# myrrix/myrrix-recommender

Hardware: AMD Instinct MI355X
Metric: ALS rows solved/sec (full iteration) at k=64 (higher is better)
Workload: dtype f32 storage; per-row Gramian: f16x2-split operands (22 bits), f32 accumulate; Cholesky f32

## Files before the change

### myrrix-recommender_amd/csrc/als_kernels.h

```cpp
#pragma once
#include <hip/hip_runtime.h>
#include <stdint.h>

#include <type_traits>

namespace mals {

#ifndef MALS_WAVES
#define MALS_WAVES(T, MODE) ((T) <= 4 ? 4 : ((T) == 5 ? 3 : 2))
#endif
#ifndef MALS_WAVES_H
#define MALS_WAVES_H(T, MODE) ((T) <= 2 ? 5 : ((T) <= 4 ? 3 : 2))
#endif

typedef float f32x4 __attribute__((ext_vector_type(4)));
typedef double f64x4 __attribute__((ext_vector_type(4)));

__host__ __device__ constexpr int tri(int T) { return T * (T + 1) / 2; }
__host__ __device__ constexpr int tidx(int T, int i, int j) { return i * T - (i * (i - 1)) / 2 + (j - i); }

constexpr int GRAMIAN_FLUSH_BINADES = 5;
constexpr int YMAX_SLOTS = 64;

struct WorkItem {
  int64_t begin;
  int32_t len;
  int32_t id;
};
struct RowC {
  int64_t first_slot;
  int32_t row;
  int32_t nseg;
  int32_t stride;
  int32_t pad_;
};
constexpr int FINISH_GROUP = 32;

struct SolveParams {
  const int64_t* row_ptr;
  const int32_t* col;
  const float* val;
  const float* M;
  const float* Gf;
  const float* Gperm;
  float* out;
  const WorkItem* items;
  const RowC* rowsC;
  float* scratch;
  unsigned long long* bad_row;
  unsigned long long* suspect;
  int* any_marked;
  uint8_t* refine_flag;
  float refine_limit;
  float gramian_weight;
  int64_t n_work;
  int32_t k;
  int32_t ldm;
  int32_t flags;
  float alpha;
  float lambda_alpha;
  float sing_threshold;
  const float* zscale;
  unsigned long long* trace;
  int trace_start;
};

__device__ __forceinline__ float bperm(int byte_idx, float v) {
  return __int_as_float(__builtin_amdgcn_ds_bpermute(byte_idx, __float_as_int(v)));
}
__device__ __forceinline__ float readlane(float v, int lane) {
  return __int_as_float(__builtin_amdgcn_readlane(__float_as_int(v), lane));
}
__device__ __forceinline__ float select4(int q, float t0, float t1, float t2, float t3) {
  const bool b0 = q & 1, b1 = q & 2;
  const float lo = b0 ? t1 : t0, hi = b0 ? t3 : t2;
  return b1 ? hi : lo;
}
__device__ __forceinline__ int uniform(int v) { return __builtin_amdgcn_readfirstlane(v); }
__device__ __forceinline__ int64_t uniform64(int64_t v) {
  const unsigned lo = (unsigned)__builtin_amdgcn_readfirstlane((int)(unsigned)(v & 0xffffffffll));
  const int hi = __builtin_amdgcn_readfirstlane((int)(v >> 32));
  return ((int64_t)hi << 32) | lo;
}
template <int N>
__device__ __forceinline__ float row_ror(float v) {
  return __int_as_float(__builtin_amdgcn_update_dpp(0, __float_as_int(v), 0x120 + N, 0xf, 0xf, false));
}
template <int LANE>
__device__ __forceinline__ float row_bcast(float v) {
  return __int_as_float(__builtin_amdgcn_update_dpp(0, __float_as_int(v), 0x150 + LANE, 0xf, 0xf, false));
}
__device__ __forceinline__ float reduce_row16(float x) {
  x += row_ror<8>(x);
  x += row_ror<4>(x);
  x += row_ror<2>(x);
  x += row_ror<1>(x);
  return x;
}
#ifndef MALS_REDUCE_GROUPS_BPERM
#define MALS_REDUCE_GROUPS_BPERM 0
#endif
__device__ __forceinline__ float reduce_groups(float x, int lane) {
#if MALS_REDUCE_GROUPS_BPERM
  x += bperm((lane ^ 16) << 2, x);
  x += bperm((lane ^ 32) << 2, x);
  return x;
#else
  typedef unsigned u32x2 __attribute__((ext_vector_type(2)));
  const unsigned xi = __float_as_uint(x);
  const u32x2 a = __builtin_amdgcn_permlane32_swap(xi, xi, false, false);
  const float s = __uint_as_float(a[0]) + __uint_as_float(a[1]);
  const unsigned si = __float_as_uint(s);
  const u32x2 b = __builtin_amdgcn_permlane16_swap(si, si, false, false);
  return __uint_as_float(b[0]) + __uint_as_float(b[1]);
#endif
}
__device__ __forceinline__ f32x4 mfma4(float a, float b, f32x4 c) {
  return __builtin_amdgcn_mfma_f32_16x16x4f32(a, b, c, 0, 0, 0);
}

__device__ __forceinline__ f32x4 tile_ptq(const f32x4& P, const f32x4& Q, f32x4 C) {
  C = mfma4(P[0], Q[0], C);
  C = mfma4(P[1], Q[1], C);
  C = mfma4(P[2], Q[2], C);
  C = mfma4(P[3], Q[3], C);
  return C;
}
__device__ __forceinline__ f32x4 tile_neg_ptq(const f32x4& P, const f32x4& Q, f32x4 C) {
  C = mfma4(-P[0], Q[0], C);
  C = mfma4(-P[1], Q[1], C);
  C = mfma4(-P[2], Q[2], C);
  C = mfma4(-P[3], Q[3], C);
  return C;
}

__device__ __forceinline__ float spread_to_col(float v, int lane);
template <int T_>
__device__ __forceinline__ void diag_step(f32x4& D, f32x4& E, int lane, int pos, float& minpiv, float& piv, float& num) {
  constexpr int gm = T_ & 3, rm = T_ >> 2, P = 4 * gm + rm;
  constexpr int gn = (T_ + 1) & 3, rn = ((T_ + 1) >> 2) & 3, PN = 4 * gn + rn;
  const int c = lane & 15;
  const float rinv = __builtin_amdgcn_rcpf(piv);
  float nl = -(num * rinv);
  nl = pos > T_ ? nl : 0.f;
#define MALS_FMAC_BCAST(n, cond) ".if " cond "\n\tv_fmac_f32_dpp %" #n ", %" #n ", %8 row_newbcast:%9 row_mask:0xf bank_mask:0xf\n\t.endif\n\t"
  if constexpr (T_ < 15) {
    asm volatile(".if %10 == 0\n\ts_nop 1\n\t.endif\n\t"
                 MALS_FMAC_BCAST(0, "%11 == 0") MALS_FMAC_BCAST(1, "%11 == 1") MALS_FMAC_BCAST(2, "%11 == 2") MALS_FMAC_BCAST(3, "%11 == 3")
                 : "+v"(D[0]), "+v"(D[1]), "+v"(D[2]), "+v"(D[3]), "+v"(E[0]), "+v"(E[1]), "+v"(E[2]), "+v"(E[3])
                 : "v"(nl), "n"(P), "n"(T_), "n"(rn));
    __builtin_amdgcn_sched_barrier(0);
    num = bperm(((16 * gn) | c) << 2, D[rn]);
    piv = readlane(D[rn], 16 * gn + PN);
    __builtin_amdgcn_sched_barrier(0);
    asm volatile(MALS_FMAC_BCAST(0, "(3 > %10) && (%11 != 0)") MALS_FMAC_BCAST(1, "(7 > %10) && (%11 != 1)")
                 MALS_FMAC_BCAST(2, "(11 > %10) && (%11 != 2)") MALS_FMAC_BCAST(3, "(15 > %10) && (%11 != 3)")
                 MALS_FMAC_BCAST(4, "0 <= %10") MALS_FMAC_BCAST(5, "4 <= %10") MALS_FMAC_BCAST(6, "8 <= %10") MALS_FMAC_BCAST(7, "12 <= %10")
                 : "+v"(D[0]), "+v"(D[1]), "+v"(D[2]), "+v"(D[3]), "+v"(E[0]), "+v"(E[1]), "+v"(E[2]), "+v"(E[3])
                 : "v"(nl), "n"(P), "n"(T_), "n"(rn));
  } else {
    asm volatile(MALS_FMAC_BCAST(4, "0 <= %10") MALS_FMAC_BCAST(5, "4 <= %10") MALS_FMAC_BCAST(6, "8 <= %10") MALS_FMAC_BCAST(7, "12 <= %10")
                 : "+v"(D[0]), "+v"(D[1]), "+v"(D[2]), "+v"(D[3]), "+v"(E[0]), "+v"(E[1]), "+v"(E[2]), "+v"(E[3])
                 : "v"(nl), "n"(P), "n"(T_), "n"(rn));
  }
#undef MALS_FMAC_BCAST
}

__device__ __forceinline__ f32x4 factor_diag(f32x4 D, int lane, float& minpiv) {
  const int g = lane >> 4, c = lane & 15;
  const int pos = 4 * (c & 3) + (c >> 2);
  f32x4 E;
#pragma unroll
  for (int r = 0; r < 4; ++r) E[r] = (4 * g + r == c) ? 1.f : 0.f;
  float num = bperm(c << 2, D[0]);
  float piv = readlane(D[0], 0);
  diag_step<0>(D, E, lane, pos, minpiv, piv, num);
  diag_step<1>(D, E, lane, pos, minpiv, piv, num);
  diag_step<2>(D, E, lane, pos, minpiv, piv, num);
  diag_step<3>(D, E, lane, pos, minpiv, piv, num);
  diag_step<4>(D, E, lane, pos, minpiv, piv, num);
  diag_step<5>(D, E, lane, pos, minpiv, piv, num);
  diag_step<6>(D, E, lane, pos, minpiv, piv, num);
  diag_step<7>(D, E, lane, pos, minpiv, piv, num);
  diag_step<8>(D, E, lane, pos, minpiv, piv, num);
  diag_step<9>(D, E, lane, pos, minpiv, piv, num);
  diag_step<10>(D, E, lane, pos, minpiv, piv, num);
  diag_step<11>(D, E, lane, pos, minpiv, piv, num);
  diag_step<12>(D, E, lane, pos, minpiv, piv, num);
  diag_step<13>(D, E, lane, pos, minpiv, piv, num);
  diag_step<14>(D, E, lane, pos, minpiv, piv, num);
  diag_step<15>(D, E, lane, pos, minpiv, piv, num);
  const float pvc = spread_to_col(select4(c & 3, D[0], D[1], D[2], D[3]), lane);
  minpiv = fminf(minpiv, pvc == pvc ? pvc : 0.f);
  const float s = __builtin_amdgcn_rsqf(pvc);
#pragma unroll
  for (int r = 0; r < 4; ++r) E[r] *= s;
  return E;
}

typedef _Float16 f16x4h __attribute__((ext_vector_type(4)));
typedef int i32x2h __attribute__((ext_vector_type(2)));
struct TileH {
  i32x2h h, l;
};
__device__ __forceinline__ int pk_rn16(float a, float b) {
  typedef float f32x2r __attribute__((ext_vector_type(2)));
  typedef _Float16 f16x2r __attribute__((ext_vector_type(2)));
  const f32x2r v = {a, b};
  return __builtin_bit_cast(int, __builtin_convertvector(v, f16x2r));
}
__device__ __forceinline__ float residual_lo(int h, float z) {
  float o;
  asm("v_fma_mix_f32 %0, %1, -1.0, %2 op_sel:[0,0,0] op_sel_hi:[1,0,0]" : "=v"(o) : "v"(h), "v"(z));
  return o;
}
__device__ __forceinline__ float residual_hi(int h, float z) {
  float o;
  asm("v_fma_mix_f32 %0, %1, -1.0, %2 op_sel:[1,0,0] op_sel_hi:[1,0,0]" : "=v"(o) : "v"(h), "v"(z));
  return o;
}

__device__ __forceinline__ TileH split_tile(const f32x4& t) {
  const int h01 = pk_rn16(t[0], t[1]), h23 = pk_rn16(t[2], t[3]);
  const int l01 = pk_rn16(residual_lo(h01, t[0]), residual_hi(h01, t[1]));
  const int l23 = pk_rn16(residual_lo(h23, t[2]), residual_hi(h23, t[3]));
  TileH o;
  o.h[0] = h01;
  o.h[1] = h23;
  o.l[0] = l01;
  o.l[1] = l23;
  return o;
}
__device__ __forceinline__ TileH negate_tile(const TileH& t) {
  TileH o;
  o.h = t.h ^ (int)0x80008000;
  o.l = t.l ^ (int)0x80008000;
  return o;
}
__device__ __forceinline__ f32x4 mfma16h(const i32x2h& a, const i32x2h& b, f32x4 c) {
  return __builtin_amdgcn_mfma_f32_16x16x16f16(__builtin_bit_cast(f16x4h, a), __builtin_bit_cast(f16x4h, b), c, 0, 0, 0);
}
__device__ __forceinline__ f32x4 tile_ptq_h(const TileH& P, const TileH& Q, f32x4 C) {
  C = mfma16h(P.h, Q.h, C);
// ... 231 lines not shown
      "ds_bpermute_b32 %0, %4, %5 offset:%7\n\t"
      "ds_bpermute_b32 %1, %4, %5 offset:%8\n\t"
      "ds_bpermute_b32 %2, %4, %6 offset:%7\n\t"
      "ds_bpermute_b32 %3, %4, %6 offset:%8\n\t"
      "s_waitcnt lgkmcnt(0)"
      : "=&v"(a0), "=&v"(a1), "=&v"(b0), "=&v"(b1)
      : "v"(addr), "v"(a), "v"(b), "n"(O0), "n"(O1));
}
template <int O0, int O1>
__device__ __forceinline__ void bperm2_i_start(int addr, int v, int& r0, int& r1) {
  asm volatile(
      "ds_bpermute_b32 %0, %2, %3 offset:%4\n\t"
      "ds_bpermute_b32 %1, %2, %3 offset:%5"
      : "=&v"(r0), "=&v"(r1)
      : "v"(addr), "v"(v), "n"(O0), "n"(O1));
}
__device__ __forceinline__ void bperm2_i_land(int& r0, int& r1) {
  asm volatile("s_waitcnt lgkmcnt(0)" : "+v"(r0), "+v"(r1));
}
template <int O0, int O1>
__device__ __forceinline__ void bperm2_i(int addr, int v, int& r0, int& r1) {
  asm volatile(
      "ds_bpermute_b32 %0, %2, %3 offset:%4\n\t"
      "ds_bpermute_b32 %1, %2, %3 offset:%5\n\t"
      "s_waitcnt lgkmcnt(0)"
      : "=&v"(r0), "=&v"(r1)
      : "v"(addr), "v"(v), "n"(O0), "n"(O1));
}

template <bool ROWMAJOR = false>
__device__ __forceinline__ Chunk chunk_issue(const SolveParams& p, int64_t begin, int len, int base, int lane) {
  const int n = base + (ROWMAJOR ? (((lane & 15) << 2) | (lane >> 4)) : lane);
  const int nn = n < len ? n : len - 1;
  Chunk e;
  e.col = __builtin_nontemporal_load(p.col + begin + nn);
  e.w = __builtin_nontemporal_load(p.val + begin + nn);
  e.cb = n < len ? 1.f : 0.f;
  return e;
}
__device__ __forceinline__ void chunk_weights(const SolveParams& p, Chunk& e) {
  const float r = e.w, ok = e.cb;
  const float base_w = (p.flags & 2) ? 1.f : 0.f;
  float w, cb;
  if (p.flags & 1) {
    w = base_w;
    cb = r;
  } else {
    const float ar = p.alpha * fabsf(r);
    w = base_w + ar;
    cb = r > 0.f ? 1.f + ar : 0.f;
  }
  e.w = ok * w;
  e.cb = ok * cb;
}

template <int T>
__device__ __forceinline__ void load_rows(const float* __restrict__ M, int ldm, int col, int c, float (&y)[T]) {
  const float* p = M + ((uint64_t)(uint32_t)col * (uint32_t)ldm + (uint32_t)c);
#pragma unroll
  for (int v = 0; v < T; ++v) y[v] = p[16 * v];
}

template <int T>
__device__ __forceinline__ void gram_step(const float (&y)[T], float w, float cb, f32x4 (&acc)[tri(T)], float (&bpart)[T]) {
  float a[T];
#pragma unroll
  for (int v = 0; v < T; ++v) a[v] = w * y[v];
#pragma unroll
  for (int i = 0; i < T; ++i)
#pragma unroll
    for (int j = i; j < T; ++j) acc[tidx(T, i, j)] = mfma4(a[i], y[j], acc[tidx(T, i, j)]);
#pragma unroll
  for (int v = 0; v < T; ++v) bpart[v] = fmaf(cb, y[v], bpart[v]);
}

template <int T, int D>
struct Pipe {
  Chunk ch;
  float y[D][T];
  float wcur, cbcur;
  int colpf;
};

template <int T, int D, bool FULL>
__device__ __forceinline__ void prime_row(const SolveParams& p, int lane, Pipe<T, D>& pp) {
  const int c = lane & 15, gb = (lane >> 4) << 2;
#pragma unroll
  for (int i = 0; i < D - 1; ++i) load_rows<T>(p.M, p.ldm, bperm_i(gb + 16 * i, pp.ch.col), c, pp.y[i]);
  pp.wcur = bperm(gb, pp.ch.w);
  pp.cbcur = bperm(gb, pp.ch.cb);
  pp.colpf = bperm_i(gb + 16 * (D - 1), pp.ch.col);
}

template <int T, int D, bool FULL>
__device__ __forceinline__ void gather_row(const SolveParams& p, int64_t begin, int len, int lane, Pipe<T, D>& pp,
                                           f32x4 (&acc)[tri(T)], float (&bpart)[T]) {
  static_assert(16 % D == 0, "ring depth must divide the chunk length in steps");
  const int c = lane & 15, gb = (lane >> 4) << 2;
  const int nsteps = (len + 3) >> 2;
  for (int q = 0; 16 * q < nsteps; ++q) {
    Chunk chn = chunk_issue(p, begin, len, 64 * (q + 1), lane);
#pragma unroll
    for (int j = 0; j < 16; ++j) {
      const int s = 16 * q + j;
      if (s < nsteps) {
        load_rows<T>(p.M, p.ldm, pp.colpf, c, pp.y[(j + D - 1) % D]);
        __builtin_amdgcn_sched_barrier(0);
        if (j == 14) chunk_weights(p, chn);
        const int jn = j + 1, jt = j + D;
        const float wn = bperm(gb + 16 * (jn & 15), jn < 16 ? pp.ch.w : chn.w);
        const float cbn = bperm(gb + 16 * (jn & 15), jn < 16 ? pp.ch.cb : chn.cb);
        const int coln = bperm_i(gb + 16 * (jt & 15), jt < 16 ? pp.ch.col : chn.col);
        gram_step<T>(pp.y[j % D], pp.wcur, pp.cbcur, acc, bpart);
        pp.wcur = wn;
        pp.cbcur = cbn;
        pp.colpf = coln;
        __builtin_amdgcn_sched_barrier(0);
      }
    }
    pp.ch = chn;
  }
}

typedef _Float16 f16x8 __attribute__((ext_vector_type(8)));
typedef _Float16 f16x4 __attribute__((ext_vector_type(4)));
typedef _Float16 f16x2 __attribute__((ext_vector_type(2)));
typedef int i32x4 __attribute__((ext_vector_type(4)));
typedef int i32x2 __attribute__((ext_vector_type(2)));

template <int E>
struct ZOp {
  int r[E / 2];
};
template <int E>
__device__ __forceinline__ f32x4 mfma_h(const ZOp<E>& a, const ZOp<E>& b, f32x4 c) {
  if constexpr (E == 8) {
    return __builtin_amdgcn_mfma_f32_16x16x32_f16(__builtin_bit_cast(f16x8, a), __builtin_bit_cast(f16x8, b), c, 0, 0, 0);
  } else {
    return __builtin_amdgcn_mfma_f32_16x16x16f16(__builtin_bit_cast(f16x4, a), __builtin_bit_cast(f16x4, b), c, 0, 0, 0);
  }
}
#ifndef MALS_SPLIT8_MAXT
#define MALS_SPLIT8_MAXT 7
#endif
__host__ __device__ constexpr int split_slots(int T) { return T <= MALS_SPLIT8_MAXT ? 8 : 4; }

__device__ __forceinline__ void chunk_weights_h(const SolveParams& p, Chunk& e, float zscale) {
  chunk_weights(p, e);
  e.w = __builtin_amdgcn_sqrtf(e.w) * zscale;
}

template <int T, int E, bool FULL, int E2>
__device__ __forceinline__ void issue_pair_h(const SolveParams& p, int col_src, int off, int lane, float (&raw)[T][E]) {
  const int c = lane & 15;
  int col[2];
  bperm2_i<8 * E2, 8 * E2 + 4>(off, col_src, col[0], col[1]);
#ifdef MALS_PROFILING
  if (p.flags & 0x400) {
    col[0] &= 0xfff;
    col[1] &= 0xfff;
  }
#endif
#pragma unroll
  for (int i = 0; i < 2; ++i) {
    const int e = 2 * E2 + i;
    const float* ptr = p.M + ((uint64_t)(uint32_t)col[i] * (uint32_t)p.ldm + (uint32_t)c);
#pragma unroll
    for (int v = 0; v < T; ++v) raw[v][e] = ptr[16 * v];
  }
}

template <int E2>
__device__ __forceinline__ void fetch_pair_cols_h(int col_src, int off, int (&col)[2]) {
  bperm2_i_start<8 * E2, 8 * E2 + 4>(off, col_src, col[0], col[1]);
}
template <int T, int E, bool FULL, int E2>
__device__ __forceinline__ void issue_pair_loads_h(const SolveParams& p, int (&col)[2], int lane, float (&raw)[T][E]) {
  const int c = lane & 15;
  bperm2_i_land(col[0], col[1]);
#ifdef MALS_PROFILING
  if (p.flags & 0x400) {
    col[0] &= 0xfff;
    col[1] &= 0xfff;
  }
#endif
#pragma unroll
  for (int i = 0; i < 2; ++i) {
    const int e = 2 * E2 + i;
    const float* ptr = p.M + ((uint64_t)(uint32_t)col[i] * (uint32_t)p.ldm + (uint32_t)c);
#pragma unroll
    for (int v = 0; v < T; ++v) raw[v][e] = ptr[16 * v];
  }
}

template <int T, int E, bool FULL, int PART, int E2, int NTERM = 2>
__device__ __forceinline__ void convert_pair_h(const SolveParams& p, const Chunk& ch, int lane, const float (&raw)[T][E], ZOp<E> (&zh)[T],
                                               ZOp<E> (&zl)[T], float (&bpart)[T], ZOp<E> (&zm)[NTERM == 3 ? T : 1]) {
  constexpr int m0 = E * PART + 2 * E2;
  const float s0 = row_bcast<m0>(ch.w), s1 = row_bcast<m0 + 1>(ch.w);
  const float c0 = row_bcast<m0>(ch.cb), c1 = row_bcast<m0 + 1>(ch.cb);
#pragma unroll
  for (int v = 0; v < T; ++v) {
    const float y0 = raw[v][2 * E2], y1 = raw[v][2 * E2 + 1];
    const float z0 = y0 * s0, z1 = y1 * s1;
    const int hp = pk_rn16(z0, z1);
    const f16x2 hh = __builtin_bit_cast(f16x2, hp);
    zh[v].r[E2] = hp;
    if constexpr (NTERM == 3) {
      const float r0 = fmaf((float)hh[0], -1.f, z0), r1 = fmaf((float)hh[1], -1.f, z1);
      const int mp = pk_rn16(r0, r1);
      const f16x2 mh = __builtin_bit_cast(f16x2, mp);
      zm[v].r[E2] = mp;
      zl[v].r[E2] = pk_rn16(fmaf((float)mh[0], -1.f, r0), fmaf((float)mh[1], -1.f, r1));
    } else {
      zl[v].r[E2] = pk_rn16(fmaf((float)hh[0], -1.f, z0), fmaf((float)hh[1], -1.f, z1));
    }
    bpart[v] = fmaf(c0, y0, bpart[v]);
    bpart[v] = fmaf(c1, y1, bpart[v]);
  }
}

template <int T, int E, bool FULL, int PART, int NTERM = 2>
__device__ __forceinline__ void convert_refill_h(const SolveParams& p, const Chunk& ch, int next_col, int next_off, int lane,
                                                 float (&raw)[T][E], ZOp<E> (&zh)[T], ZOp<E> (&zl)[T], float (&bpart)[T], ZOp<E> (&zm)[NTERM == 3 ? T : 1]) {
#define MALS_SB __builtin_amdgcn_sched_barrier(0)
  int col[2];
  fetch_pair_cols_h<0>(next_col, next_off, col);
  MALS_SB;
  convert_pair_h<T, E, FULL, PART, 0, NTERM>(p, ch, lane, raw, zh, zl, bpart, zm);
  MALS_SB;
  issue_pair_loads_h<T, E, FULL, 0>(p, col, lane, raw);
  fetch_pair_cols_h<1>(next_col, next_off, col);
  MALS_SB;
  convert_pair_h<T, E, FULL, PART, 1, NTERM>(p, ch, lane, raw, zh, zl, bpart, zm);
  MALS_SB;
  issue_pair_loads_h<T, E, FULL, 1>(p, col, lane, raw);
  if constexpr (E == 8) {
    fetch_pair_cols_h<2>(next_col, next_off, col);
    MALS_SB;
    convert_pair_h<T, E, FULL, PART, 2, NTERM>(p, ch, lane, raw, zh, zl, bpart, zm);
    MALS_SB;
    issue_pair_loads_h<T, E, FULL, 2>(p, col, lane, raw);
    fetch_pair_cols_h<3>(next_col, next_off, col);
    MALS_SB;
    convert_pair_h<T, E, FULL, PART, 3, NTERM>(p, ch, lane, raw, zh, zl, bpart, zm);
    MALS_SB;
    issue_pair_loads_h<T, E, FULL, 3>(p, col, lane, raw);
  }
#undef MALS_SB
}

template <int T, int E>
__device__ __forceinline__ void gram_super_step(const ZOp<E> (&zh)[T], const ZOp<E> (&zl)[T], f32x4 (&acc)[tri(T)]) {
#pragma unroll
  for (int i = 0; i < T; ++i)
#pragma unroll
    for (int j = i; j < T; ++j) acc[tidx(T, i, j)] = mfma_h<E>(zh[i], zh[j], acc[tidx(T, i, j)]);
#pragma unroll
  for (int i = 0; i < T; ++i)
#pragma unroll
    for (int j = i; j < T; ++j) acc[tidx(T, i, j)] = mfma_h<E>(zh[i], zl[j], acc[tidx(T, i, j)]);
#pragma unroll
  for (int i = 0; i < T; ++i)
#pragma unroll
    for (int j = i; j < T; ++j) acc[tidx(T, i, j)] = mfma_h<E>(zl[i], zh[j], acc[tidx(T, i, j)]);
}

template <int T, int E>
__device__ __forceinline__ void gram_super_step3(const ZOp<E> (&zh)[T], const ZOp<E> (&zm)[T], const ZOp<E> (&zl)[T], f32x4 (&acc)[tri(T)]) {
#define MALS_GS3(A, B)                                                                                    \
  _Pragma("unroll") for (int i = 0; i < T; ++i) _Pragma("unroll") for (int j = i; j < T; ++j)              \
      acc[tidx(T, i, j)] = mfma_h<E>(A[i], B[j], acc[tidx(T, i, j)])
  MALS_GS3(zl, zh);
  MALS_GS3(zh, zl);
  MALS_GS3(zm, zm);
  MALS_GS3(zm, zh);
  MALS_GS3(zh, zm);
  MALS_GS3(zh, zh);
#undef MALS_GS3
}

template <int T, int E, bool FULL>
__device__ __forceinline__ void prime_row_h(const SolveParams& p, int col_src, int lane, float (&raw)[T][E]) {
  const int rb = (lane & 48) << 2;
  issue_pair_h<T, E, FULL, 0>(p, col_src, rb, lane, raw);
  issue_pair_h<T, E, FULL, 1>(p, col_src, rb, lane, raw);
  if constexpr (E == 8) {
    issue_pair_h<T, E, FULL, 2>(p, col_src, rb, lane, raw);
    issue_pair_h<T, E, FULL, 3>(p, col_src, rb, lane, raw);
  }
}

template <int T, int E, bool FULL, int PART, int NTERM = 2>
__device__ __forceinline__ void super_step_h(const SolveParams& p, const Chunk& ch, const Chunk& chn, int next_col, bool last, int lane,
                                             float (&raw)[T][E], f32x4 (&acc)[tri(T)], float (&bpart)[T]) {
  constexpr int NP = 16 / E;
  const int rb = (lane & 48) << 2;
  ZOp<E> zh[T], zl[T], zm[NTERM == 3 ? T : 1];
  const int same_row_col = PART == NP - 1 ? chn.col : ch.col;
  const int same_row_off = PART == NP - 1 ? rb : rb + 4 * E * (PART + 1);
  convert_refill_h<T, E, FULL, PART, NTERM>(p, ch, last ? next_col : same_row_col, last ? rb : same_row_off, lane, raw, zh, zl, bpart, zm);
  __builtin_amdgcn_sched_barrier(0);
  if constexpr (NTERM == 3) gram_super_step3<T, E>(zh, zm, zl, acc);
  else gram_super_step<T, E>(zh, zl, acc);
  __builtin_amdgcn_sched_barrier(0);
}

template <int T, int E, bool FULL, int NTERM = 2>
__device__ __forceinline__ void gather_row_h(const SolveParams& p, int64_t begin, int len, int lane, float zscale, Chunk& ch,
                                             int next_col, float (&raw)[T][E], f32x4 (&acc)[tri(T)], float (&bpart)[T]) {
  constexpr int NS = 4 * E, NP = 16 / E;
  const int n_ss = (len + NS - 1) / NS;
  for (int q = 0; NP * q < n_ss; ++q) {
    Chunk chn = chunk_issue<true>(p, begin, len, 64 * (q + 1), lane);
    const int ss = NP * q;
    super_step_h<T, E, FULL, 0, NTERM>(p, ch, chn, next_col, ss + 1 >= n_ss, lane, raw, acc, bpart);
    if (ss + 1 < n_ss) {
      if (NP == 2) chunk_weights_h(p, chn, zscale);
      super_step_h<T, E, FULL, 1, NTERM>(p, ch, chn, next_col, ss + 2 >= n_ss, lane, raw, acc, bpart);
    }
    if constexpr (NP == 4) {
      if (ss + 2 < n_ss) super_step_h<T, E, FULL, 2, NTERM>(p, ch, chn, next_col, ss + 3 >= n_ss, lane, raw, acc, bpart);
      if (ss + 3 < n_ss) {
        chunk_weights_h(p, chn, zscale);
        super_step_h<T, E, FULL, 3, NTERM>(p, ch, chn, next_col, ss + 4 >= n_ss, lane, raw, acc, bpart);
      }
    }
    ch = chn;
  }
}

template <int T>
__device__ __forceinline__ void init_acc(const SolveParams& p, f32x4 (&acc)[tri(T)], int lane) {
  if (!(p.flags & 2)) {
    const f32x4* G4 = reinterpret_cast<const f32x4*>(p.Gf) + lane;
#pragma unroll
    for (int t = 0; t < tri(T); ++t) acc[t] = G4[t * 64];
  } else {
#pragma unroll
    for (int t = 0; t < tri(T); ++t) acc[t] = f32x4{0.f, 0.f, 0.f, 0.f};
  }
}

template <int T, bool FULL = false>
__device__ __forceinline__ void add_ridge(const SolveParams& p, f32x4 (&acc)[tri(T)], int n_u, int lane) {
  const int g = lane >> 4, c = lane & 15;
  const float ridge = p.lambda_alpha * (float)n_u;
  float rd[4];
#pragma unroll
  for (int r = 0; r < 4; ++r) rd[r] = (4 * g + r == c) ? ridge : 0.f;
  float w00 = 1.f;
  if constexpr (!FULL) w00 = readlane(acc[tidx(T, 0, 0)][0], 0) + ridge;
#pragma unroll
  for (int v = 0; v < T; ++v) {
    if (FULL || v < T - 1) {
#pragma unroll
      for (int r = 0; r < 4; ++r) acc[tidx(T, v, v)][r] += rd[r];
    } else {
      const int feat = 16 * v + c;
#pragma unroll
      for (int r = 0; r < 4; ++r) {
        if (4 * g + r == c) acc[tidx(T, v, v)][r] = feat < p.k ? acc[tidx(T, v, v)][r] + ridge : w00;
      }
    }
  }
}

__device__ __forceinline__ int wave_max_bits(float mf, int lane) {
  int m = __float_as_int(mf);
  m = max(m, __builtin_amdgcn_update_dpp(0, m, 0x120 + 8, 0xf, 0xf, false));
  m = max(m, __builtin_amdgcn_update_dpp(0, m, 0x120 + 4, 0xf, 0xf, false));
  m = max(m, __builtin_amdgcn_update_dpp(0, m, 0x120 + 2, 0xf, 0xf, false));
  m = max(m, __builtin_amdgcn_update_dpp(0, m, 0x120 + 1, 0xf, 0xf, false));
  m = max(m, bperm_i((lane ^ 16) << 2, m));
  m = max(m, bperm_i((lane ^ 32) << 2, m));
  return m;
}
template <int T>
__device__ __forceinline__ int max_entry_bits(const f32x4 (&acc)[tri(T)], int lane) {
  float mf = 0.f;
#pragma unroll
  for (int v = 0; v < T; ++v) {
    const f32x4& d = acc[tidx(T, v, v)];
    mf = fmaxf(mf, fmaxf(fmaxf(fabsf(d[0]), fabsf(d[1])), fmaxf(fabsf(d[2]), fabsf(d[3]))));
  }
  return wave_max_bits(mf, lane);
}

template <int T>
__device__ __forceinline__ float row_part_max(const f32x4 (&acc)[tri(T)], const f32x4* gimg, int lane) {
  float mf = 0.f;
#pragma unroll
  for (int v = 0; v < T; ++v) {
    const f32x4 d = acc[tidx(T, v, v)] - gimg[tidx(T, v, v) * 64 + lane];
    mf = fmaxf(mf, fmaxf(fmaxf(fabsf(d[0]), fabsf(d[1])), fmaxf(fabsf(d[2]), fabsf(d[3]))));
  }
  return __int_as_float(wave_max_bits(mf, lane));
}

#ifndef MALS_PK_MAXT
#define MALS_PK_MAXT 7
#endif
template <int T>
__device__ __forceinline__ float row_scale(f32x4 (&acc)[tri(T)], float (&bcol)[T], int lane, float& wmax) {
  const int m = max_entry_bits<T>(acc, lane);
  wmax = __int_as_float(m);
  const int e = ((m >> 23) & 255) - 126;
  int p2 = 2 * (13 - ((e + 1) >> 1));
  p2 = p2 < -100 ? -100 : (p2 > 100 ? 100 : p2);
  const float s2 = __int_as_float((p2 + 127) << 23), inv_s2 = __int_as_float((127 - p2) << 23);
#pragma unroll
  for (int t = 0; t < tri(T); ++t) {
    if constexpr (T <= MALS_PK_MAXT) {
      acc[t] = acc[t] * s2;
    } else {
#pragma unroll
      for (int r = 0; r < 4; ++r) acc[t][r] *= s2;
    }
  }
#pragma unroll
  for (int v = 0; v < T; ++v) bcol[v] *= s2;
  return inv_s2;
}

template <int T, bool PERM = false>
__device__ __forceinline__ void store_row(const SolveParams& p, float (&xcol)[T], float minpiv, float wmax, int row, int lane) {
  if (!(minpiv > p.sing_threshold)) {
    if (lane == 0) {
      if (p.refine_flag) {
        p.refine_flag[row] = 2;
        *p.any_marked = 1;
      } else {
        atomicMin(p.bad_row, (unsigned long long)row);
      }
    }
#pragma unroll
    for (int v = 0; v < T; ++v) xcol[v] = 0.f;
  } else {
    if (minpiv <= 1024.f * p.sing_threshold && lane == 0) {
      const unsigned long long key = ((unsigned long long)__float_as_uint(minpiv) << 32) | (unsigned)row;
      if (key < __builtin_nontemporal_load(p.suspect)) atomicMin(p.suspect, key);
    }
    if (p.refine_flag && p.refine_limit > 0.f && wmax > p.refine_limit * minpiv && lane == 0) {
      p.refine_flag[row] = 1;
      *p.any_marked = 1;
    }
  }
  if constexpr (PERM) {
    static_assert(T == 8, "the permuted feature order belongs to the k = 128 kernels");
    float* o = p.out + (int64_t)row * p.k;
    int l2 = lane;
    asm volatile("" : "+v"(l2));
    const int g = l2 >> 4, c = l2 & 15;
    const bool hi = ((g ^ (c >> 3)) & 1) != 0;
    f32x4 x;
#pragma unroll
    for (int q = 0; q < 4; ++q) x[q] = hi ? xcol[4 + q] : xcol[q];
    if (g < 2) *reinterpret_cast<f32x4*>(o + 8 * c + 4 * g) = x;
  } else {
    float* o = p.out + (int64_t)row * p.k;
    int l2 = lane;
    asm volatile("" : "+v"(l2));
    const int g = l2 >> 4, c = l2 & 15;
#pragma unroll
    for (int m = 0; 4 * m < T; ++m) {
      const float x = select4(g, xcol[4 * m], 4 * m + 1 < T ? xcol[4 * m + 1] : 0.f, 4 * m + 2 < T ? xcol[4 * m + 2] : 0.f,
                              4 * m + 3 < T ? xcol[4 * m + 3] : 0.f);
      const int feat = 16 * (4 * m + g) + c;
      if (4 * m + 3 < T - 1 || feat < p.k) o[feat] = x;
    }
  }
}

template <int T, bool PERM = false>
__device__ __forceinline__ void finish_row(const SolveParams& p, f32x4 (&acc)[tri(T)], const float (&bcol)[T],
                                           int n_u, int row, int lane, float rmax = 0.f) {
  add_ridge<T, PERM>(p, acc, n_u, lane);
  float minpiv = 3.0e38f;
  float xcol[T];
  const float wmax = fmaxf(rmax, p.gramian_weight * __int_as_float(max_entry_bits<T>(acc, lane)));
  cholesky_tiles<T>(acc, lane, minpiv);
  solve_tiles<T>(acc, bcol, xcol, lane);
  store_row<T, PERM>(p, xcol, minpiv, wmax, row, lane);
}

__device__ __forceinline__ WorkItem load_item(const SolveParams& p, int64_t it) {
  WorkItem w;
  if (it < p.n_work) {
    w = p.items[it];
  } else {
    w.begin = 0;
    w.len = -1;
    w.id = 0;
  }
  return w;
}

template <int T, int D, int MODE, bool FULL>
__global__ __launch_bounds__(256, MALS_WAVES(T, MODE)) void als_persistent_kernel(SolveParams p) {
  __shared__ f32x4 sG[MODE == 0 ? tri(T) * 64 : 1];
  const int lane = threadIdx.x & 63;
  const int wave = uniform(blockIdx.x * 4 + (threadIdx.x >> 6));
  const int64_t n_waves = (int64_t)gridDim.x * 4;
  if (MODE == 0) {
    const f32x4* G4 = reinterpret_cast<const f32x4*>(p.Gf);
    for (int e = threadIdx.x; e < tri(T) * 64; e += 256) sG[e] = (p.flags & 2) ? f32x4{0.f, 0.f, 0.f, 0.f} : G4[e];
    __syncthreads();
  }
  int64_t it = wave;
  if (it >= p.n_work) return;
  if ((p.flags & 8) && p.zscale[2] != 0.f) return;
  WorkItem cur = load_item(p, it);
  WorkItem nxt = load_item(p, it + n_waves);
  Pipe<T, D> pp;
  pp.wcur = pp.cbcur = 0.f;
  pp.colpf = 0;
  pp.ch.col = 0;
  pp.ch.w = pp.ch.cb = 0.f;
#pragma unroll
  for (int i = 0; i < D; ++i)
#pragma unroll
    for (int v = 0; v < T; ++v) pp.y[i][v] = 0.f;
  if (cur.len > 0) {
    pp.ch = chunk_issue(p, cur.begin, cur.len, 0, lane);
    chunk_weights(p, pp.ch);
    prime_row<T, D, FULL>(p, lane, pp);
  }
  for (;;) {
    f32x4 acc[tri(T)];
    if (MODE == 0) {
#pragma unroll
      for (int t = 0; t < tri(T); ++t) acc[t] = sG[t * 64 + lane];
    } else {
#pragma unroll
      for (int t = 0; t < tri(T); ++t) acc[t] = f32x4{0.f, 0.f, 0.f, 0.f};
    }
    float bpart[T];
#pragma unroll
    for (int v = 0; v < T; ++v) bpart[v] = 0.f;
#ifdef MALS_PROFILING
    const int64_t trow = it / n_waves - p.trace_start;
    const bool tr = MODE == 0 && p.trace && wave < 64 && trow >= 0 && trow < 64;
    unsigned long long t0 = 0, t1 = 0, t2 = 0, t3 = 0;
    if (tr) t0 = __builtin_readcyclecounter();
    if (!(p.flags & 0x200)) gather_row<T, D, FULL>(p, cur.begin, cur.len, lane, pp, acc, bpart);
    if (tr) t1 = __builtin_readcyclecounter();
#else
    gather_row<T, D, FULL>(p, cur.begin, cur.len, lane, pp, acc, bpart);
#endif
    float bcol[T];
#pragma unroll
    for (int v = 0; v < T; ++v) bcol[v] = reduce_groups(bpart[v], lane);
    const bool prime_next = nxt.len > 0;
    if (prime_next) pp.ch = chunk_issue(p, nxt.begin, nxt.len, 0, lane);
    const WorkItem nxt2 = load_item(p, it + 2 * n_waves);
    if (MODE == 0) {
      const float wmax = p.refine_flag ? fmaxf(row_part_max<T>(acc, sG, lane), p.gramian_weight * __int_as_float(max_entry_bits<T>(acc, lane))) : 0.f;
      add_ridge<T, FULL>(p, acc, cur.len, lane);
      float minpiv = 3.0e38f;
      float xcol[T];
#ifdef MALS_PROFILING
      if (p.flags & 0x100) {
#pragma unroll
        for (int v = 0; v < T; ++v) xcol[v] = 1e-3f + 1e-9f * (bcol[v] + acc[tidx(T, v, v)][0] + acc[tidx(T, 0, v)][1]);
        if (prime_next) {
          chunk_weights(p, pp.ch);
          prime_row<T, D, FULL>(p, lane, pp);
        }
      } else
#endif
      {
        cholesky_tiles<T>(acc, lane, minpiv);
#ifdef MALS_PROFILING
        if (tr) t2 = __builtin_readcyclecounter();
#endif
        if (prime_next) {
          chunk_weights(p, pp.ch);
          prime_row<T, D, FULL>(p, lane, pp);
        }
        solve_tiles<T>(acc, bcol, xcol, lane);
      }
      store_row<T>(p, xcol, minpiv, wmax, cur.id, lane);
#ifdef MALS_PROFILING
      if (tr) {
        t3 = __builtin_readcyclecounter();
        if (lane == 0) {
          unsigned long long* o = p.trace + (trow * 64 + wave) * 6;
          o[0] = t0; o[1] = t1; o[2] = t2; o[3] = t3; o[4] = (unsigned long long)cur.len; o[5] = wall_clock64();
        }
      }
#endif
    } else {
      float* s = p.scratch + (int64_t)cur.id * ((tri(T) * 4 + T) * 64);
#pragma unroll
      for (int t = 0; t < tri(T); ++t) reinterpret_cast<f32x4*>(s)[t * 64 + lane] = acc[t];
#pragma unroll
      for (int v = 0; v < T; ++v) s[(tri(T) * 4 + v) * 64 + lane] = bcol[v];
      if (prime_next) {
        chunk_weights(p, pp.ch);
        prime_row<T, D, FULL>(p, lane, pp);
      }
    }
    if (nxt.len < 0) break;
    cur = nxt;
    nxt = nxt2;
    it += n_waves;
  }
}

template <int T, int MODE, bool FULL, int NTERM = 2>
__global__ __launch_bounds__(256, MALS_WAVES_H(T, MODE)) void als_persistent_kernel_h(SolveParams p) {
  __shared__ f32x4 sG[MODE == 0 ? tri(T) * 64 : 1];
  const int lane = threadIdx.x & 63;
  const int wave = uniform(blockIdx.x * 4 + (threadIdx.x >> 6));
  const int64_t n_waves = (int64_t)gridDim.x * 4;
  if (MODE == 0) {
    const f32x4* G4 = reinterpret_cast<const f32x4*>(p.Gf);
    for (int e = threadIdx.x; e < tri(T) * 64; e += 256) sG[e] = (p.flags & 2) ? f32x4{0.f, 0.f, 0.f, 0.f} : G4[e];
    __syncthreads();
  }
  int64_t it = wave;
  if (it >= p.n_work) return;
  if (p.zscale[2] == 0.f) return;
  const float zscale = __int_as_float(uniform(__float_as_int(p.zscale[0])));
  const float inv_s2 = __int_as_float(uniform(__float_as_int(p.zscale[1])));
  WorkItem cur = load_item(p, it);
  WorkItem nxt = load_item(p, it + n_waves);
  WorkItem nx2 = load_item(p, it + 2 * n_waves);
  constexpr int E = split_slots(T);
  float raw[T][E];
#pragma unroll
  for (int v = 0; v < T; ++v)
#pragma unroll
    for (int e = 0; e < E; ++e) raw[v][e] = 0.f;
  if (cur.len > 0) {
    Chunk ch = chunk_issue<true>(p, cur.begin, cur.len, 0, lane);
    Chunk nch = nxt.len > 0 ? chunk_issue<true>(p, nxt.begin, nxt.len, 0, lane) : ch;
    chunk_weights_h(p, ch, zscale);
    prime_row_h<T, E, FULL>(p, ch.col, lane, raw);
    for (;;) {
      const WorkItem nx3 = load_item(p, it + 3 * n_waves);
      f32x4 acc[tri(T)];
#pragma unroll
      for (int t = 0; t < tri(T); ++t) acc[t] = f32x4{0.f, 0.f, 0.f, 0.f};
      float bpart[T];
#pragma unroll
      for (int v = 0; v < T; ++v) bpart[v] = 0.f;
#ifdef MALS_PROFILING
      const int64_t trow = it / n_waves - p.trace_start;
      const bool tr = MODE == 0 && p.trace && wave < 64 && trow >= 0 && trow < 64;
      unsigned long long t0 = 0, t1 = 0, t2 = 0;
      if (tr) t0 = __builtin_readcyclecounter();
#endif
      gather_row_h<T, E, FULL, NTERM>(p, cur.begin, cur.len, lane, zscale, ch, nch.col, raw, acc, bpart);
#ifdef MALS_PROFILING
      if (tr) t1 = __builtin_readcyclecounter();
#endif
      float bcol[T];
#pragma unroll
      for (int v = 0; v < T; ++v) bcol[v] = reduce_groups(bpart[v], lane);
      ch = nch;
      if (nxt.len > 0) chunk_weights_h(p, ch, zscale);
      if (MODE == 0) {
        const float rmax = p.refine_flag ? __int_as_float(max_entry_bits<T>(acc, lane)) * inv_s2 : 0.f;
#pragma unroll
        for (int t = 0; t < tri(T); ++t) {
          const f32x4 g4 = sG[t * 64 + lane];
          if constexpr (T <= MALS_PK_MAXT) {
            acc[t] = __builtin_elementwise_fma(acc[t], f32x4{inv_s2, inv_s2, inv_s2, inv_s2}, g4);
          } else {
#pragma unroll
            for (int r = 0; r < 4; ++r) acc[t][r] = fmaf(acc[t][r], inv_s2, g4[r]);
          }
        }
        add_ridge<T, FULL>(p, acc, cur.len, lane);
        float minpiv = 3.0e38f, wmax;
        float xcol[T];
        if constexpr (T >= 2) {
          const float inv_s2row = row_scale<T>(acc, bcol, lane, wmax);
          cholesky_tiles<T, true>(acc, lane, minpiv);
          minpiv *= inv_s2row;
        } else {
          wmax = __int_as_float(max_entry_bits<T>(acc, lane));
          cholesky_tiles<T>(acc, lane, minpiv);
        }
#ifdef MALS_PROFILING
        if (tr) t2 = __builtin_readcyclecounter();
#endif
        solve_tiles<T>(acc, bcol, xcol, lane);
        store_row<T>(p, xcol, minpiv, fmaxf(rmax, p.gramian_weight * wmax), cur.id, lane);
#ifdef MALS_PROFILING
        if (tr) {
          const unsigned long long t3 = __builtin_readcyclecounter();
          if (lane == 0) {
            unsigned long long* o = p.trace + (trow * 64 + wave) * 6;
            o[0] = t0; o[1] = t1; o[2] = t2; o[3] = t3; o[4] = (unsigned long long)cur.len; o[5] = wall_clock64();
          }
        }
#endif
      } else {
        float* s = p.scratch + (int64_t)cur.id * ((tri(T) * 4 + T) * 64);
#pragma unroll
        for (int t = 0; t < tri(T); ++t) reinterpret_cast<f32x4*>(s)[t * 64 + lane] = acc[t] * inv_s2;
#pragma unroll
        for (int v = 0; v < T; ++v) s[(tri(T) * 4 + v) * 64 + lane] = bcol[v];
      }
      cur = nxt;
      nxt = nx2;
      nx2 = nx3;
      nch = nxt.len > 0 ? chunk_issue<true>(p, nxt.begin, nxt.len, 0, lane) : nch;
      it += n_waves;
      if (cur.len <= 0) break;
    }
  }
  if (MODE == 0) {
    while (cur.len == 0) {
      f32x4 acc[tri(T)];
#pragma unroll
      for (int t = 0; t < tri(T); ++t) acc[t] = sG[t * 64 + lane];
      float bcol[T];
#pragma unroll
      for (int v = 0; v < T; ++v) bcol[v] = 0.f;
      finish_row<T>(p, acc, bcol, 0, cur.id, lane);
      it += n_waves;
      cur = load_item(p, it);
    }
  }
}

template <int T>
__device__ __forceinline__ void add_slot(const float* __restrict__ s, int lane, f32x4 (&acc)[tri(T)], float (&bcol)[T]) {
  constexpr int PASSES = T >= 6 ? 2 : 1, PER = (tri(T) + PASSES - 1) / PASSES;
#pragma unroll
  for (int ps = 0; ps < PASSES; ++ps) {
    f32x4 part[PER];
#pragma unroll
    for (int t = 0; t < PER; ++t)
      if (ps * PER + t < tri(T)) part[t] = reinterpret_cast<const f32x4*>(s)[(ps * PER + t) * 64 + lane];
    if (ps == 0) {
      float bp[T];
#pragma unroll
      for (int v = 0; v < T; ++v) bp[v] = s[(tri(T) * 4 + v) * 64 + lane];
#pragma unroll
      for (int v = 0; v < T; ++v) bcol[v] += bp[v];
    }
#pragma unroll
    for (int t = 0; t < PER; ++t)
      if (ps * PER + t < tri(T)) acc[ps * PER + t] += part[t];
    if (PASSES > 1) __builtin_amdgcn_sched_barrier(0);
  }
}

template <int T>
__global__ __launch_bounds__(256) void als_prereduce_kernel(SolveParams p) {
  const int lane = threadIdx.x & 63;
  const int64_t wave = (int64_t)blockIdx.x * 4 + (threadIdx.x >> 6);
  if (wave >= p.n_work) return;
  RowC rc = p.rowsC[wave];
  rc.first_slot = uniform64(rc.first_slot);
  rc.nseg = uniform(rc.nseg);
  constexpr int SLOT = (tri(T) * 4 + T) * 64;
  float* s0 = p.scratch + rc.first_slot * (int64_t)SLOT;
  f32x4 acc[tri(T)];
  float bcol[T];
#pragma unroll
  for (int t = 0; t < tri(T); ++t) acc[t] = reinterpret_cast<const f32x4*>(s0)[t * 64 + lane];
#pragma unroll
  for (int v = 0; v < T; ++v) bcol[v] = s0[(tri(T) * 4 + v) * 64 + lane];
  for (int sgi = 1; sgi < rc.nseg; ++sgi) {
    add_slot<T>(s0 + sgi * (int64_t)SLOT, lane, acc, bcol);
  }
#pragma unroll
  for (int t = 0; t < tri(T); ++t) reinterpret_cast<f32x4*>(s0)[t * 64 + lane] = acc[t];
#pragma unroll
  for (int v = 0; v < T; ++v) s0[(tri(T) * 4 + v) * 64 + lane] = bcol[v];
}

template <int T, bool PERM = false>
__global__ __launch_bounds__(256, T >= 6 ? 2 : 1) void als_finish_kernel(SolveParams p) {
  const int lane = threadIdx.x & 63;
  const int64_t wave = (int64_t)blockIdx.x * 4 + (threadIdx.x >> 6);
  if (wave >= p.n_work) return;
  if (PERM && p.zscale[2] == 0.f) return;
  if (!PERM && (p.flags & 8) && p.zscale[2] != 0.f) return;
  RowC rc = p.rowsC[wave];
  rc.first_slot = uniform64(rc.first_slot);
  rc.row = uniform(rc.row);
  rc.nseg = uniform(rc.nseg);
  rc.stride = uniform(rc.stride);
  f32x4 acc[tri(T)];
#pragma unroll
  for (int t = 0; t < tri(T); ++t) acc[t] = f32x4{0.f, 0.f, 0.f, 0.f};
  float bcol[T];
#pragma unroll
  for (int v = 0; v < T; ++v) bcol[v] = 0.f;
  for (int sgi = 0; sgi < rc.nseg; ++sgi) {
    const float* s = p.scratch + (rc.first_slot + (int64_t)sgi * rc.stride) * (int64_t)((tri(T) * 4 + T) * 64);
    add_slot<T>(s, lane, acc, bcol);
  }
  const int n_u = uniform((int)(p.row_ptr[rc.row + 1] - p.row_ptr[rc.row]));
  const float rmax = p.refine_flag ? __int_as_float(max_entry_bits<T>(acc, lane)) : 0.f;
  if (!(p.flags & 2)) {
    const f32x4* G4 = reinterpret_cast<const f32x4*>(PERM ? p.Gperm : p.Gf) + lane;
#pragma unroll
    for (int t = 0; t < tri(T); ++t) acc[t] += G4[t * 64];
  }
  finish_row<T, PERM>(p, acc, bcol, n_u, rc.row, lane, rmax);
// ... 773 lines not shown
```

Baseline: 138.3 million.

## Skip gather loads and conversions for padded slot pairs in short split rows

Adds a per-super-step count of live slot pairs and, for MODE 1 with T<=4 and 8-slot splitting, skips the column fetches, global loads and f16 split conversions for pairs that are entirely padding, zeroing their operands instead. This targets wasted memory traffic and ALU work on short rows whose tail chunk is mostly padding. It also switches row_bcast to mov_dpp, precomputes a byte base pointer for the gather addresses, and folds the residual computation into a single fma from the raw value. The extra branches are wave-uniform but add control flow, and the fused residual changes rounding slightly.

```diff
diff --git a/myrrix-recommender_amd/csrc/als_kernels.h b/myrrix-recommender_amd/csrc/als_kernels.h
--- a/myrrix-recommender_amd/csrc/als_kernels.h
+++ b/myrrix-recommender_amd/csrc/als_kernels.h
@@ -88,7 +88,7 @@
 }
 template <int LANE>
 __device__ __forceinline__ float row_bcast(float v) {
-  return __int_as_float(__builtin_amdgcn_update_dpp(0, __float_as_int(v), 0x150 + LANE, 0xf, 0xf, false));
+  return __int_as_float(__builtin_amdgcn_mov_dpp(__float_as_int(v), 0x150 + LANE, 0xf, 0xf, false));
 }
 __device__ __forceinline__ float reduce_row16(float x) {
   x += row_ror<8>(x);
@@ -626,7 +626,7 @@
 
 template <int T, int E, bool FULL, int E2>
 __device__ __forceinline__ void issue_pair_h(const SolveParams& p, int col_src, int off, int lane, float (&raw)[T][E]) {
-  const int c = lane & 15;
+  const char* gbase = reinterpret_cast<const char*>(p.M + (lane & 15));
   int col[2];
   bperm2_i<8 * E2, 8 * E2 + 4>(off, col_src, col[0], col[1]);
 #ifdef MALS_PROFILING
@@ -638,7 +638,7 @@
 #pragma unroll
   for (int i = 0; i < 2; ++i) {
     const int e = 2 * E2 + i;
-    const float* ptr = p.M + ((uint64_t)(uint32_t)col[i] * (uint32_t)p.ldm + (uint32_t)c);
+    const float* ptr = reinterpret_cast<const float*>(gbase + (uint64_t)(uint32_t)col[i] * (uint32_t)(p.ldm << 2));
 #pragma unroll
     for (int v = 0; v < T; ++v) raw[v][e] = ptr[16 * v];
   }
@@ -650,7 +650,7 @@
 }
 template <int T, int E, bool FULL, int E2>
 __device__ __forceinline__ void issue_pair_loads_h(const SolveParams& p, int (&col)[2], int lane, float (&raw)[T][E]) {
-  const int c = lane & 15;
+  const char* gbase = reinterpret_cast<const char*>(p.M + (lane & 15));
   bperm2_i_land(col[0], col[1]);
 #ifdef MALS_PROFILING
   if (p.flags & 0x400) {
@@ -661,7 +661,7 @@
 #pragma unroll
   for (int i = 0; i < 2; ++i) {
     const int e = 2 * E2 + i;
-    const float* ptr = p.M + ((uint64_t)(uint32_t)col[i] * (uint32_t)p.ldm + (uint32_t)c);
+    const float* ptr = reinterpret_cast<const float*>(gbase + (uint64_t)(uint32_t)col[i] * (uint32_t)(p.ldm << 2));
 #pragma unroll
     for (int v = 0; v < T; ++v) raw[v][e] = ptr[16 * v];
   }
@@ -681,46 +681,47 @@
     const f16x2 hh = __builtin_bit_cast(f16x2, hp);
     zh[v].r[E2] = hp;
     if constexpr (NTERM == 3) {
-      const float r0 = fmaf((float)hh[0], -1.f, z0), r1 = fmaf((float)hh[1], -1.f, z1);
+      const float r0 = fmaf(y0, s0, -(float)hh[0]), r1 = fmaf(y1, s1, -(float)hh[1]);
       const int mp = pk_rn16(r0, r1);
       const f16x2 mh = __builtin_bit_cast(f16x2, mp);
       zm[v].r[E2] = mp;
       zl[v].r[E2] = pk_rn16(fmaf((float)mh[0], -1.f, r0), fmaf((float)mh[1], -1.f, r1));
     } else {
-      zl[v].r[E2] = pk_rn16(fmaf((float)hh[0], -1.f, z0), fmaf((float)hh[1], -1.f, z1));
+      zl[v].r[E2] = pk_rn16(fmaf(y0, s0, -(float)hh[0]), fmaf(y1, s1, -(float)hh[1]));
     }
     bpart[v] = fmaf(c0, y0, bpart[v]);
     bpart[v] = fmaf(c1, y1, bpart[v]);
   }
 }
 
+template <int T, int E, int E2, int NTERM>
+__device__ __forceinline__ void zero_pair_h(ZOp<E> (&zh)[T], ZOp<E> (&zl)[T], ZOp<E> (&zm)[NTERM == 3 ? T : 1]) {
+#pragma unroll
+  for (int v = 0; v < T; ++v) {
+    zh[v].r[E2] = 0;
+    zl[v].r[E2] = 0;
+    if constexpr (NTERM == 3) zm[v].r[E2] = 0;
+  }
+}
 template <int T, int E, bool FULL, int PART, int NTERM = 2>
-__device__ __forceinline__ void convert_refill_h(const SolveParams& p, const Chunk& ch, int next_col, int next_off, int lane,
+__device__ __forceinline__ void convert_refill_h(const SolveParams& p, const Chunk& ch, int next_col, int next_off, int live, int next_live, int lane,
                                                  float (&raw)[T][E], ZOp<E> (&zh)[T], ZOp<E> (&zl)[T], float (&bpart)[T], ZOp<E> (&zm)[NTERM == 3 ? T : 1]) {
 #define MALS_SB __builtin_amdgcn_sched_barrier(0)
+#define MALS_PAIR(E2)                                                                  \
+  if (E2 == 0 || next_live > E2) fetch_pair_cols_h<E2>(next_col, next_off, col);       \
+  MALS_SB;                                                                             \
+  if (E2 == 0 || live > E2) convert_pair_h<T, E, FULL, PART, E2, NTERM>(p, ch, lane, raw, zh, zl, bpart, zm); \
+  else zero_pair_h<T, E, E2, NTERM>(zh, zl, zm);                                       \
+  MALS_SB;                                                                             \
+  if (E2 == 0 || next_live > E2) issue_pair_loads_h<T, E, FULL, E2>(p, col, lane, raw)
   int col[2];
-  fetch_pair_cols_h<0>(next_col, next_off, col);
-  MALS_SB;
-  convert_pair_h<T, E, FULL, PART, 0, NTERM>(p, ch, lane, raw, zh, zl, bpart, zm);
-  MALS_SB;
-  issue_pair_loads_h<T, E, FULL, 0>(p, col, lane, raw);
-  fetch_pair_cols_h<1>(next_col, next_off, col);
-  MALS_SB;
-  convert_pair_h<T, E, FULL, PART, 1, NTERM>(p, ch, lane, raw, zh, zl, bpart, zm);
-  MALS_SB;
-  issue_pair_loads_h<T, E, FULL, 1>(p, col, lane, raw);
+  MALS_PAIR(0);
+  MALS_PAIR(1);
   if constexpr (E == 8) {
-    fetch_pair_cols_h<2>(next_col, next_off, col);
-    MALS_SB;
-    convert_pair_h<T, E, FULL, PART, 2, NTERM>(p, ch, lane, raw, zh, zl, bpart, zm);
-    MALS_SB;
-    issue_pair_loads_h<T, E, FULL, 2>(p, col, lane, raw);
-    fetch_pair_cols_h<3>(next_col, next_off, col);
-    MALS_SB;
-    convert_pair_h<T, E, FULL, PART, 3, NTERM>(p, ch, lane, raw, zh, zl, bpart, zm);
-    MALS_SB;
-    issue_pair_loads_h<T, E, FULL, 3>(p, col, lane, raw);
-  }
+    MALS_PAIR(2);
+    MALS_PAIR(3);
+  }
+#undef MALS_PAIR
 #undef MALS_SB
 }
 
@@ -755,53 +756,65 @@
 }
 
 template <int T, int E, bool FULL>
-__device__ __forceinline__ void prime_row_h(const SolveParams& p, int col_src, int lane, float (&raw)[T][E]) {
+__device__ __forceinline__ void prime_row_h(const SolveParams& p, int col_src, int live, int lane, float (&raw)[T][E]) {
   const int rb = (lane & 48) << 2;
   issue_pair_h<T, E, FULL, 0>(p, col_src, rb, lane, raw);
-  issue_pair_h<T, E, FULL, 1>(p, col_src, rb, lane, raw);
+  if (live > 1) issue_pair_h<T, E, FULL, 1>(p, col_src, rb, lane, raw);
   if constexpr (E == 8) {
-    issue_pair_h<T, E, FULL, 2>(p, col_src, rb, lane, raw);
-    issue_pair_h<T, E, FULL, 3>(p, col_src, rb, lane, raw);
+    if (live > 2) issue_pair_h<T, E, FULL, 2>(p, col_src, rb, lane, raw);
+    if (live > 3) issue_pair_h<T, E, FULL, 3>(p, col_src, rb, lane, raw);
   }
 }
 
 template <int T, int E, bool FULL, int PART, int NTERM = 2>
-__device__ __forceinline__ void super_step_h(const SolveParams& p, const Chunk& ch, const Chunk& chn, int next_col, bool last, int lane,
+__device__ __forceinline__ void super_step_h(const SolveParams& p, const Chunk& ch, const Chunk& chn, int next_col, bool last, int live, int next_live, int lane,
                                              float (&raw)[T][E], f32x4 (&acc)[tri(T)], float (&bpart)[T]) {
   constexpr int NP = 16 / E;
   const int rb = (lane & 48) << 2;
   ZOp<E> zh[T], zl[T], zm[NTERM == 3 ? T : 1];
   const int same_row_col = PART == NP - 1 ? chn.col : ch.col;
   const int same_row_off = PART == NP - 1 ? rb : rb + 4 * E * (PART + 1);
-  convert_refill_h<T, E, FULL, PART, NTERM>(p, ch, last ? next_col : same_row_col, last ? rb : same_row_off, lane, raw, zh, zl, bpart, zm);
+  convert_refill_h<T, E, FULL, PART, NTERM>(p, ch, last ? next_col : same_row_col, last ? rb : same_row_off, live, next_live, lane, raw, zh, zl, bpart, zm);
   __builtin_amdgcn_sched_barrier(0);
   if constexpr (NTERM == 3) gram_super_step3<T, E>(zh, zm, zl, acc);
   else gram_super_step<T, E>(zh, zl, acc);
   __builtin_amdgcn_sched_barrier(0);
 }
 
-template <int T, int E, bool FULL, int NTERM = 2>
+__host__ __device__ constexpr bool skips_padding(int T, int MODE) { return MODE == 1 && T <= 4 && split_slots(T) == 8; }
+template <int E, bool SKIP>
+__device__ __forceinline__ int live_pairs(int n) {
+  if constexpr (!SKIP) return E / 2;
+  return n >= 4 * E ? E / 2 : (n + 7) >> 3;
+}
+
+template <int T, int E, bool FULL, int NTERM = 2, bool SKIP = false>
 __device__ __forceinline__ void gather_row_h(const SolveParams& p, int64_t begin, int len, int lane, float zscale, Chunk& ch,
-                                             int next_col, float (&raw)[T][E], f32x4 (&acc)[tri(T)], float (&bpart)[T]) {
+                                             int next_col, int next_len, float (&raw)[T][E], f32x4 (&acc)[tri(T)], float (&bpart)[T]) {
   constexpr int NS = 4 * E, NP = 16 / E;
   const int n_ss = (len + NS - 1) / NS;
+  const int next_row_live = live_pairs<E, SKIP>(next_len);
+#define MALS_SS(PART)                                                                                                  \
+  super_step_h<T, E, FULL, PART, NTERM>(p, ch, chn, next_col, ss + PART + 1 >= n_ss, live_pairs<E, SKIP>(len - NS * (ss + PART)), \
+                                        ss + PART + 1 >= n_ss ? next_row_live : live_pairs<E, SKIP>(len - NS * (ss + PART + 1)), lane, raw, acc, bpart)
   for (int q = 0; NP * q < n_ss; ++q) {
     Chunk chn = chunk_issue<true>(p, begin, len, 64 * (q + 1), lane);
     const int ss = NP * q;
-    super_step_h<T, E, FULL, 0, NTERM>(p, ch, chn, next_col, ss + 1 >= n_ss, lane, raw, acc, bpart);
+    MALS_SS(0);
     if (ss + 1 < n_ss) {
       if (NP == 2) chunk_weights_h(p, chn, zscale);
-      super_step_h<T, E, FULL, 1, NTERM>(p, ch, chn, next_col, ss + 2 >= n_ss, lane, raw, acc, bpart);
+      MALS_SS(1);
     }
     if constexpr (NP == 4) {
-      if (ss + 2 < n_ss) super_step_h<T, E, FULL, 2, NTERM>(p, ch, chn, next_col, ss + 3 >= n_ss, lane, raw, acc, bpart);
+      if (ss + 2 < n_ss) MALS_SS(2);
       if (ss + 3 < n_ss) {
         chunk_weights_h(p, chn, zscale);
-        super_step_h<T, E, FULL, 3, NTERM>(p, ch, chn, next_col, ss + 4 >= n_ss, lane, raw, acc, bpart);
+        MALS_SS(3);
       }
     }
     ch = chn;
   }
+#undef MALS_SS
 }
 
 template <int T>
@@ -1102,6 +1115,7 @@
   WorkItem nxt = load_item(p, it + n_waves);
   WorkItem nx2 = load_item(p, it + 2 * n_waves);
   constexpr int E = split_slots(T);
+  constexpr bool SKIP = skips_padding(T, MODE);
   float raw[T][E];
 #pragma unroll
   for (int v = 0; v < T; ++v)
@@ -1111,7 +1125,7 @@
     Chunk ch = chunk_issue<true>(p, cur.begin, cur.len, 0, lane);
     Chunk nch = nxt.len > 0 ? chunk_issue<true>(p, nxt.begin, nxt.len, 0, lane) : ch;
     chunk_weights_h(p, ch, zscale);
-    prime_row_h<T, E, FULL>(p, ch.col, lane, raw);
+    prime_row_h<T, E, FULL>(p, ch.col, live_pairs<E, SKIP>(cur.len), lane, raw);
     for (;;) {
       const WorkItem nx3 = load_item(p, it + 3 * n_waves);
       f32x4 acc[tri(T)];
@@ -1126,7 +1140,7 @@
       unsigned long long t0 = 0, t1 = 0, t2 = 0;
       if (tr) t0 = __builtin_readcyclecounter();
 #endif
-      gather_row_h<T, E, FULL, NTERM>(p, cur.begin, cur.len, lane, zscale, ch, nch.col, raw, acc, bpart);
+      gather_row_h<T, E, FULL, NTERM, SKIP>(p, cur.begin, cur.len, lane, zscale, ch, nch.col, nxt.len, raw, acc, bpart);
 #ifdef MALS_PROFILING
       if (tr) t1 = __builtin_readcyclecounter();
 #endif
```

Result: faster. 139.8 million, median of 6 (+1.1%).
